# jimahlstrom/quisk

Hardware: AMD Instinct MI355X
Metric: Mcomplex-samples/s through RXA chain (higher is better)
Workload: dtype f64; 1 GPU; 256 channels/GPU x 192 kHz IQ -> 48 kHz SSB RXA chain (shift + 561-tap resample/4 + adc meter + NBP nc 2048 + S meter + fixed AGC + agc meter + panel), 2^22 input samples per channel per step; meters=on, ingest=f64, channels_per_gpu=256, total_channels=256, dsp_size=256, parallelism=channel-sharded x1 (weak), no collective

## Files before the change

### quisk_amd/csrc/qh_engine.hip

```cpp
#include <hip/hip_runtime.h>
#include <algorithm>
#include <cmath>
#include <cstdarg>
#include <cstdio>
#include <cstdlib>
#include <cstring>
#include <map>
#include <mutex>
#include <string>
#include <vector>
#include "../../include/quiskhip.h"
#include "qh_design.hpp"
#include "qh_kernels.hpp"
#include "qh_demod.hpp"
#include "qh_tiled.hpp"
#include "qh_agc_tiled.hpp"
#include "qh_emnr.hpp"
#include "qh_snba.hpp"
#include "qh_audio_peak.hpp"
#include "qh_ssql.hpp"
#include "qh_internal.hpp"

namespace qh {

thread_local std::string g_last_error;

int set_error(int code, const char *fmt, ...)
{
    char buf[512];
    va_list ap;
    va_start(ap, fmt);
    vsnprintf(buf, sizeof(buf), fmt, ap);
    va_end(ap);
    g_last_error = buf;
    return code;
}

static constexpr int kNfft = 4096;
static constexpr int kBandNfftMax = 8192;
static constexpr int kHistBand = 4095;
static constexpr int kLongPart = 4096, kLongNcMax = 65536, kLongParts = kLongNcMax / kLongPart, kLongHist = kLongNcMax - 1;
static constexpr int kHistFront = 2240;
static constexpr int kFmTile = 256;
static constexpr int kFmWarm = 768;
static constexpr int kSamTile = 4096;
static constexpr int kSamWarm = 8192;
static constexpr long long kSamTiledMin = 4 * 8192;
static constexpr int kAgcSegs = 16;
static constexpr long long kAgcTiledMin = 16384;

struct ChanCfg {
    int mode = QH_LSB;
    int shift_run = 1; double shift_freq = 0.0;
    int shift_on_device = 1;
    int nbp_run = 1, nbp_nc = 2048, nbp_wintype = 0;
    int mp = 0;
    std::vector<Notch> notches;
    double ndb_tunefreq = 0.0, ndb_shift = 0.0;
    int fnfrun = 0, autoincr = 1;
    double nbp_flow = -4150.0, nbp_fhigh = -150.0, nbp_gain = 1.0;
    int amd_run = 0, amd_mode = 0, fmd_run = 0;
// ... 395 lines not shown
    std::vector<cd> tw = fft_twiddle_table(kNfft);
    if (int rc = alloc(tw4096, (long long)tw.size())) return rc;
    if (int rc = upload(tw4096, tw, stream)) return rc;
    tw = fft_twiddle_table(kBandNfftMax);
    if (int rc = alloc(tw8192, (long long)tw.size())) return rc;
    if (int rc = upload(tw8192, tw, stream)) return rc;

    if (D > 1) {
        ResamplerDesign rd = design_resampler(in_rate, dsp_rate, 0.0, 0, 1.0);
        if (rd.L != 1 || rd.M != D) return set_error(QH_ERR_UNSUPPORTED, "resampler L/M = %d/%d not supported", rd.L, rd.M);
        front_ntaps = rd.ncoef;
        front_fold = D > 8 ? 8 : D;
        front_pick = D / front_fold;
        front_P = ((front_ntaps - 1 + front_fold - 1) / front_fold) * front_fold;
        front_L = (((kNfft - front_P) / front_fold) / front_pick) * front_pick;
        if (front_P > kHistFront) return set_error(QH_ERR_UNSUPPORTED, "resampler history %d too long", front_P);
        if (int rc = alloc(mask_front, (long long)nch * kNfft)) return rc;
        if (int rc = alloc(lane_rot, (long long)nch * NT)) return rc;
        if (int rc = alloc(front_taps, front_ntaps)) return rc;
        if (int rc = alloc(retune_list, nch)) return rc;
        if (int rc = alloc(retune_law, 2LL * nch)) return rc;
        QH_HIP(hipMemcpyAsync(front_taps, rd.h.data(), (size_t)front_ntaps * sizeof(double), hipMemcpyHostToDevice, stream));
        QH_HIP(hipStreamSynchronize(stream));
        QH_HIP(hipFuncSetAttribute(reinterpret_cast<const void *>(&front_mask_kernel<kNfft>), hipFuncAttributeMaxDynamicSharedMemorySize,
                                   (TileFft<kNfft, false, double2>::kLdsBytes)));
        std::vector<cd> twi = fft_twiddle_table(kNfft / front_fold);
        if (int rc = alloc(tw_inv_front, (long long)twi.size())) return rc;
        if (int rc = upload(tw_inv_front, twi, stream)) return rc;
        for (double2 *&h : hist_front) if (int rc = alloc(h, (long long)nch * kHistFront, true)) return rc;
    }
    if (int rc = alloc(mask_nbp, (long long)nch * kBandNfftMax)) return rc;
    if (int rc = alloc(mask_bp1, (long long)nch * kBandNfftMax)) return rc;
    for (int i = 0; i < 2; i++) {
        if (int rc = alloc(hist_nbp[i], (long long)nch * kHistBand, true)) return rc;
        if (int rc = alloc(hist_bp1[i], (long long)nch * kHistBand, true)) return rc;
    }
    if (int rc = alloc(nco_phase, nch, true)) return rc;
    if (int rc = alloc(nco_dphase, nch, true)) return rc;
    if (int rc = alloc(nco_parked, nch, true)) return rc;
    if (int rc = alloc(nco_step, nch)) return rc;
    if (int rc = alloc(epi, nch)) return rc;

#define QH_SET_LDS(D, ...) QH_HIP(hipFuncSetAttribute(reinterpret_cast<const void *>(&osfir_kernel<double, 4096, D, __VA_ARGS__>), \
                                                     hipFuncAttributeMaxDynamicSharedMemorySize, (osfir_lds_bytes<double, 4096, D, true>())))
    QH_SET_LDS(1, false); QH_SET_LDS(1, false, false, true);
    QH_SET_LDS(1, false, false, false, false, true); QH_SET_LDS(1, false, false, true, false, true);
#define QH_SET_LDS8(...) QH_HIP(hipFuncSetAttribute(reinterpret_cast<const void *>(&osfir_kernel<double, kBandNfftMax, 1, false, false, __VA_ARGS__>), \
                                                     hipFuncAttributeMaxDynamicSharedMemorySize, (osfir_lds_bytes<double, kBandNfftMax, 1, true>())))
    QH_SET_LDS8(false, false, false); QH_SET_LDS8(true, false, false); QH_SET_LDS8(false, false, true); QH_SET_LDS8(true, false, true);
#undef QH_SET_LDS8
#define QH_SET_LDS6K(...) QH_HIP(hipFuncSetAttribute(reinterpret_cast<const void *>(&osfir6k_kernel<__VA_ARGS__>), \
        hipFuncAttributeMaxDynamicSharedMemorySize, osfir6k_lds_bytes()))
    QH_SET_LDS6K(false, false); QH_SET_LDS6K(true, false); QH_SET_LDS6K(false, true); QH_SET_LDS6K(true, true);
#undef QH_SET_LDS6K
#define QH_SET_LDS2G(...) QH_HIP(hipFuncSetAttribute(reinterpret_cast<const void *>(&osfir8k_kernel<__VA_ARGS__>), \
                                                      hipFuncAttributeMaxDynamicSharedMemorySize, osfir8k_lds_bytes()))
    QH_SET_LDS2G(false, false); QH_SET_LDS2G(true, false); QH_SET_LDS2G(false, true); QH_SET_LDS2G(true, true);
#undef QH_SET_LDS2G
    QH_SET_LDS(2, false, false, false, true, false, true); QH_SET_LDS(4, false, false, false, true, false, true); QH_SET_LDS(8, false, false, false, true, false, true);
    QH_SET_LDS(2, false, true, false, true, false, true); QH_SET_LDS(4, false, true, false, true, false, true); QH_SET_LDS(8, false, true, false, true, false, true);
#undef QH_SET_LDS
    QH_HIP(hipStreamSynchronize(stream));
    return QH_OK;
}

static unsigned long long turns_fx(double f, double rate)
// ... 99 lines not shown
                } else {
                    h.assign(1, cd(1.0, 0.0));
                }
                last_bp1_h = h;
                if ((int)h.size() > kLongPart) h.resize((size_t)kLongPart);
                last_bp1 = band_mask(h);
                last_bp1_cfg = &c;
            }
            if (long_parts[1] > 1) if (int rc = long_masks_upload(1, ch, last_bp1_h)) return rc;
            if (int rc = put_mask(mask_bp1, ch, last_bp1)) return rc;
            c.bp1_dirty = false;
            lists_dirty = true;
        }
        if (c.nbp_flush) {
            if (int rc = zero_rows(hist_nbp, lhist[0], ch)) return rc;
            c.nbp_flush = false;
        }
        if (c.bp1_flush) {
            if (int rc = zero_rows(hist_bp1, lhist[1], ch)) return rc;
            c.bp1_flush = false;
        }
    }
    if (!nco_list.empty())
        hipLaunchKernelGGL((front_mask_kernel<kNfft>), dim3((unsigned)nco_list.size()), dim3(NT), (size_t)(TileFft<kNfft, false, double2>::kLdsBytes),
                           stream, (const double *)front_taps, front_ntaps, (const unsigned long long *)nco_dphase, (const int *)retune_list, front_fold,
                           (const double2 *)tw4096, mask_front, lane_rot, nco_step, 1);
    return QH_OK;
}

std::vector<cd> Engine::notched(const ChanCfg &c, double f_low, double f_high, double scale) const
{
    const double offset = c.ndb_tunefreq + c.ndb_shift;
    const double minwidth = (c.nbp_wintype == 1 ? 2200.0 : 1600.0) / (c.nbp_nc / 256) * ((double)dsp_rate / 48000);
    std::vector<std::pair<double, double>> bands = make_nbp(c.notches, minwidth, c.autoincr, f_low + offset, f_high + offset, nullptr);
    for (auto &b : bands) { b.first -= offset; b.second -= offset; }
    return fir_mbandpass(c.nbp_nc, bands, (double)dsp_rate, scale, c.nbp_wintype);
}

int Engine::snb_mask(ChanCfg &c, int ch)
{
    double f_low = 0.0, f_high = 0.0;
    int run_notches = 0;
    switch (c.mode) {
    case QH_LSB: case QH_CWL: case QH_DIGL: f_low = -5700.0; f_high = -250.0; run_notches = c.fnfrun; break;
    case QH_USB: case QH_CWU: case QH_DIGU: f_low = 250.0; f_high = 5700.0; run_notches = c.fnfrun; break;
    case QH_AM: case QH_SAM: case QH_DSB: case QH_FM: f_low = 250.0; f_high = 5700.0; break;
    default: break;
// ... 660 lines not shown
    QH_HIP(hipMemcpyAsync(emnr_GG, h_GG.data(), h_GG.size() * 8, hipMemcpyHostToDevice, stream));
    QH_HIP(hipMemcpyAsync(emnr_GGS, h_GGS.data(), h_GGS.size() * 8, hipMemcpyHostToDevice, stream));
    QH_HIP(hipMemcpyAsync(emnr_zeta, h_zeta.data(), h_zeta.size() * 8, hipMemcpyHostToDevice, stream));
    QH_HIP(hipMemcpyAsync(emnr_zeta_true, h_zeta_true.data(), h_zeta_true.size() * 4, hipMemcpyHostToDevice, stream));
    QH_HIP(hipStreamSynchronize(stream));
    QH_HIP(hipFuncSetAttribute(reinterpret_cast<const void *>(&emnr_kernel), hipFuncAttributeMaxDynamicSharedMemorySize, emnr_lds_bytes()));
    for (ChanCfg &c : cfg) { c.emnr_dirty = true; c.emnr_flush = false; }
    return QH_OK;
}

int Engine::ensure_buffers(long long n_mid)
{
    if (n_mid <= buf_cap) return QH_OK;
    if (int rc = quiesce()) return rc;
    for (double2 *&b : buf)
        if (int rc = alloc(b, n_mid * nch)) return rc;
    buf_cap = n_mid;
    return QH_OK;
}

std::vector<cd> Engine::band_mask(const std::vector<cd> &h) const
{
    std::vector<cd> m = make_mask(h, bnfft);
    if (!band2g) return m;
    std::vector<cd> p(m.size());
    const size_t half = m.size() / 2;
    for (size_t k = 0; k < half; k++) { p[k] = m[2 * k]; p[half + k] = m[2 * k + 1]; }
    return p;
}

int Engine::ensure_meter_partials(long long n_mid, int lout)
{
    const long long need = ((n_mid + lout - 1) / lout) * (lout / 64);
    if (need <= m_part_cap) return QH_OK;
    if (int rc = quiesce()) return rc;
    for (double2 *&m : m_part)
        if (int rc = alloc(m, need * nch)) return rc;
    m_part_cap = need;
    return QH_OK;
}

int Engine::ensure_abuf(long long n)
{
    return grow(abuf, abuf_cap, n, nch);
}

// ... 5 lines not shown
}

void Engine::tick(int cat)
{
    if (!timing) return;
    if (ev_used >= (int)ev.size()) {
        hipEvent_t e;
        (void)hipEventCreate(&e);
        ev.push_back(e);
        ev_cat.push_back(0);
    }
    ev_cat[(size_t)ev_used] = cat;
    (void)hipEventRecord(ev[(size_t)ev_used], stream);
    ev_used++;
}

template <int D, bool MIX, bool PACKED = false, bool METER = false, bool OUTMIX = false, bool EGRESS = false, int NFFT = kNfft, bool POLY = false,
          int DET = 0, bool PAIR = false>
static void launch_osfir(OsfirArgs<double> a, int ntiles, int nch, hipStream_t s)
{
    a.ntiles = ntiles;
    dim3 grid((unsigned)ntiles * (unsigned)nch), block(NT);
    constexpr int lds = osfir_lds_bytes<double, NFFT, D, METER>();
    hipLaunchKernelGGL((osfir_kernel<double, NFFT, D, MIX, PACKED, METER, OUTMIX, EGRESS, POLY, DET, PAIR>), grid, block, lds, s, a);
}
template <int NFFT>
static void launch_band(OsfirArgs<double> a, int ntiles, int nch, hipStream_t s, bool meter, bool egress)
{
    if (meter && egress) launch_osfir<1, false, false, true, false, true, NFFT>(a, ntiles, nch, s);
    else if (meter) launch_osfir<1, false, false, true, false, false, NFFT>(a, ntiles, nch, s);
    else if (egress) launch_osfir<1, false, false, false, false, true, NFFT>(a, ntiles, nch, s);
    else launch_osfir<1, false, false, false, false, false, NFFT>(a, ntiles, nch, s);
}

static void launch_band6k(OsfirArgs<double> a, int ntiles, int nch, hipStream_t s, bool meter, bool egress)
{
    a.ntiles = ntiles;
    dim3 grid((unsigned)ntiles * (unsigned)nch), block(kOsfir6kThreads);
    constexpr int lds = osfir6k_lds_bytes();
    if (meter && egress) hipLaunchKernelGGL((osfir6k_kernel<true, true>), grid, block, lds, s, a);
    else if (meter) hipLaunchKernelGGL((osfir6k_kernel<true, false>), grid, block, lds, s, a);
    else if (egress) hipLaunchKernelGGL((osfir6k_kernel<false, true>), grid, block, lds, s, a);
    else hipLaunchKernelGGL((osfir6k_kernel<false, false>), grid, block, lds, s, a);
}

static void launch_band2g(OsfirArgs<double> a, int ntiles, int nch, hipStream_t s, bool meter, bool egress)
{
// ... 2193 lines not shown
```

### quisk_amd/csrc/qh_fft.hpp

```cpp
#pragma once
#include <hip/hip_runtime.h>

namespace qh {

static constexpr double kThetaZeroMark = 8.0;


constexpr int NT = 256;

template <typename T> struct cplx_of;
template <> struct cplx_of<double> { using type = double2; };
template <> struct cplx_of<float>  { using type = float2; };
template <typename T> using cplx = typename cplx_of<T>::type;

template <typename T> __device__ __forceinline__ cplx<T> mk(T x, T y) { cplx<T> r; r.x = x; r.y = y; return r; }
template <typename C> __device__ __forceinline__ C cadd(C a, C b) { C r; r.x = a.x + b.x; r.y = a.y + b.y; return r; }
template <typename C> __device__ __forceinline__ C csub(C a, C b) { C r; r.x = a.x - b.x; r.y = a.y - b.y; return r; }
template <typename C> __device__ __forceinline__ C cmul(C a, C b)
{
    C r;
    r.x = a.x * b.x - a.y * b.y;
    r.y = a.x * b.y + a.y * b.x;
    return r;
}
__device__ __forceinline__ void lds_barrier()
{
    __builtin_amdgcn_fence(__ATOMIC_RELEASE, "workgroup", "local");
    __builtin_amdgcn_s_barrier();
    __builtin_amdgcn_fence(__ATOMIC_ACQUIRE, "workgroup", "local");
}

template <typename C> __device__ __forceinline__ C cconj(C a) { C r; r.x = a.x; r.y = -a.y; return r; }
template <bool INV, typename C> __device__ __forceinline__ C mul_mi(C a)
{
    C r;
    if (INV) { r.x = -a.y; r.y = a.x; } else { r.x = a.y; r.y = -a.x; }
    return r;
}

__device__ __forceinline__ constexpr double cos32(int a)
{
    constexpr double t[9] = { 1.0, 0.98078528040323044913, 0.92387953251128675613, 0.83146961230254523708,
                              0.70710678118654752440, 0.55557023301960222474, 0.38268343236508977173,
                              0.19509032201612826785, 0.0 };
    return t[a];
}

template <int R, int I, bool INV, typename C> __device__ __forceinline__ C mul_wconst(C a)
{
    using T = decltype(a.x);
    constexpr int A = I * (32 / R);
    if constexpr (A == 0) {
// ... 77 lines not shown
    for (int r = 2; r < R; r++) {
        if (r & 1) { wo = cmul(wo, w2); x[r] = cmul(x[r], wo); }
        else { x[r] = cmul(x[r], we); if (r + 2 < R) we = cmul(we, w2); }
    }
}

template <int N, int R, int Ns, bool INV, typename C, bool LEAN = false>
__device__ __forceinline__ int stockham_butterfly(C (&x)[R], int j, C w1)
{
    int k = j & (Ns - 1);
    if constexpr (Ns > 1) { if constexpr (LEAN) apply_twiddle_powers_lean<R>(x, w1); else apply_twiddle_powers<R>(x, w1); }
    Dft<R, INV, C>::run(x);
    return (j - k) * R + k;
}

template <int Ns, bool INV, typename C>
__device__ __forceinline__ C pass_twiddle(const C *__restrict__ tw_pass, int j)
{
    C w = tw_pass[j & (Ns - 1)];
    return INV ? cconj(w) : w;
}

template <int N, int R, bool INV, typename C>
__device__ __forceinline__ void pass_regs_to_lds(C (&x)[R], C *lds)
{
    static_assert(R == N / NT, "first pass radix must equal N/NT");
    const int j = threadIdx.x;
    Dft<R, INV, C>::run(x);
    if constexpr (16 % R == 0) {
        C *p = lds + lds_phys(j * R);
#pragma unroll
        for (int r = 0; r < R; r++) p[r] = x[r];
    } else {
        static_assert(R % 16 == 0, "first pass radix: a divisor or a multiple of 16");
        C *p = lds + lds_phys(j * R);
#pragma unroll
        for (int r = 0; r < R; r++) p[r + r / 16] = x[r];
    }
}

template <int N, int R> struct PassGeom {
    static constexpr int NB = N / R;
    static constexpr int PER = (NB + NT - 1) / NT;
};

template <int N, int R, int Ns, bool INV, typename C>
__device__ __forceinline__ void pass_lds_to_lds(C *lds, const C (&w1)[PassGeom<N, R>::PER])
{
    constexpr int NB = PassGeom<N, R>::NB;
    constexpr int PER = PassGeom<N, R>::PER;
    C x[PER][R];
    int base[PER];
    static_assert(NB % 16 == 0, "pass geometry");
#pragma unroll
    for (int p = 0; p < PER; p++) {
        int j = threadIdx.x + p * NT;
        if (NB >= NT || j < NB) {
            const C *q = lds + lds_phys(j);
#pragma unroll
            for (int r = 0; r < R; r++) x[p][r] = q[r * (NB + NB / 16)];
        }
    }
// ... 106 lines not shown
#pragma unroll
        for (int r = 0; r < 16; r++) x[r].y = rp[r * RS];
    }

    static __device__ __forceinline__ void run(C (&x)[16], void *lds_raw, const Tw &t) { run_at(x, lds_raw, t, threadIdx.x); }
    template <bool LEAN = false>
    static __device__ __forceinline__ void run_at(C (&x)[16], void *lds_raw, const Tw &t, int j)
    {
        T *lds = reinterpret_cast<T *>(lds_raw);
        Dft<16, INV, C>::run(x);
        if constexpr (kSwizzle) exchange_sw<1>(x, lds, j, 0);
        else exchange<1, 256 + 16 * kPad>(x, lds, (16 + kPad) * j, sphys(j));
        const int base = stockham_butterfly<4096, 16, 16, INV, C, LEAN>(x, j, t.a[0]);
        __syncthreads();
        if constexpr (kSwizzle) exchange_sw<2>(x, lds, j, base);
        else exchange<16 + kPad, 256 + 16 * kPad>(x, lds, sphys(base), sphys(j));
        stockham_butterfly<4096, 16, 256, INV, C, LEAN>(x, j, t.b);
    }

    template <int D>
    static __device__ __forceinline__ void run_poly(C (&x)[16], void *lds_raw, const Tw &t)
    {
        static_assert(!INV && (D == 2 || D == 4 || D == 8), "forward transform of a decimating stage");
        constexpr int R3 = 16 / D;
        const int j = threadIdx.x;
        T *lds = reinterpret_cast<T *>(lds_raw);
        Dft<16, INV, C>::run(x);
        if constexpr (kSwizzle) exchange_sw<1>(x, lds, j, 0);
        else exchange<1, 256 + 16 * kPad>(x, lds, (16 + kPad) * j, sphys(j));
        const int base = stockham_butterfly<4096, 16, 16, INV>(x, j, t.a[0]);
        __syncthreads();
        if constexpr (kSwizzle) exchange_sw<2>(x, lds, j, base);
        else exchange<16 + kPad, 256 + 16 * kPad>(x, lds, sphys(base), sphys(j));
        C w[R3];
        w[1] = t.b;
#pragma unroll
        for (int s = 1; s < D; s <<= 1) w[1] = cmul(w[1], w[1]);
#pragma unroll
        for (int r = 2; r < R3; r++) w[r] = (r & 1) ? cmul(w[r - 1], w[1]) : cmul(w[r / 2], w[r / 2]);
        C y[16];
#pragma unroll
        for (int a = 0; a < D; a++) {
            C b[R3];
            b[0] = x[a];
#pragma unroll
            for (int r = 1; r < R3; r++) b[r] = cmul(x[a + D * r], w[r]);
            Dft<R3, INV, C>::run(b);
#pragma unroll
            for (int r = 0; r < R3; r++) y[r + R3 * a] = b[r];
        }
#pragma unroll
        for (int r = 0; r < 16; r++) x[r] = y[r];
    }
};

constexpr int kFft6kThreads = 384;
constexpr int kFft6kPad = 2;
constexpr int kFft6kLdsBytes = (6144 + 6144 / 16 * kFft6kPad) * 8;

template <bool INV, typename C> __device__ __forceinline__ void dft3(C &a, C &b, C &c)
{
    const double h = 0.86602540378443864676;
    const C t1 = cadd(b, c);
    C t2; t2.x = a.x - 0.5 * t1.x; t2.y = a.y - 0.5 * t1.y;
    const C d = csub(b, c);
    C t3;
    if (INV) { t3.x = -h * d.y; t3.y = h * d.x; } else { t3.x = h * d.y; t3.y = -h * d.x; }
    a = cadd(a, t1);
    b = cadd(t2, t3);
    c = csub(t2, t3);
}

template <int M, bool INV, typename C> __device__ __forceinline__ C mul_w24(C a)
{
    constexpr int m = M % 24;
// ... 99 lines not shown
        }
        __syncthreads();
        if (mid) {
#pragma unroll
            for (int r = 0; r < 24; r++) w2[r * (16 + kPad)] = y[r].x;
        }
        __syncthreads();
        const double *r2 = lds + sphys(t);
#pragma unroll
        for (int r = 0; r < 16; r++) x[r].x = r2[r * (384 + 24 * kPad)];
        __syncthreads();
        if (mid) {
#pragma unroll
            for (int r = 0; r < 24; r++) w2[r * (16 + kPad)] = y[r].y;
        }
        __syncthreads();
#pragma unroll
        for (int r = 0; r < 16; r++) x[r].y = r2[r * (384 + 24 * kPad)];
        apply_twiddle_powers<16>(x, tw.last);
        Dft<16, INV, C>::run(x);
    }
};

template <int N, bool INV, typename C> struct TileFft {
    static constexpr bool kSplit = N == 4096 && sizeof(C) == 16;
    static constexpr int kLdsBytes = kSplit ? split4096_lds_bytes(8) : lds_elems<N>() * (int)sizeof(C);
    using Tw = typename FftRR<N, INV, C>::Tw;
    static __device__ __forceinline__ Tw load(const C *__restrict__ tw) { return FftRR<N, INV, C>::load(tw); }
    static __device__ __forceinline__ void run(C (&x)[N / NT], void *lds, const Tw &t)
    {
        if constexpr (kSplit) {
            FftSplit4096<INV, C>::run(x, lds, t);
        } else {
            FftRR<N, INV, C>::first(x, reinterpret_cast<C *>(lds));
            FftRR<N, INV, C>::rest(reinterpret_cast<C *>(lds), x, t);
        }
    }
    template <int D> static __device__ __forceinline__ void run_poly(C (&x)[N / NT], void *lds, const Tw &t)
    {
        static_assert(kSplit, "polyphase plan: the fp64 4096-point transform");
        FftSplit4096<INV, C>::template run_poly<D>(x, lds, t);
    }
};

template <bool INV, typename C> struct FftRR<2048, INV, C> {
    struct Tw { C a[2], b[1], c; };
    static __device__ __forceinline__ Tw load(const C *__restrict__ tw)
    {
        Tw t;
        t.a[0] = pass_twiddle<8, INV>(tw, threadIdx.x);
        t.a[1] = pass_twiddle<8, INV>(tw, threadIdx.x + NT);
        t.b[0] = pass_twiddle<32, INV>(tw + 8, threadIdx.x);
        t.c = pass_twiddle<256, INV>(tw + 40, threadIdx.x);
        return t;
    }
    static __device__ __forceinline__ void first(C (&x)[8], C *lds) { pass_regs_to_lds<2048, 8, INV>(x, lds); }
    static __device__ __forceinline__ void rest(C *lds, C (&x)[8], const Tw &t)
    {
        __syncthreads();
        pass_lds_to_lds<2048, 4, 8, INV>(lds, t.a);
        __syncthreads();
        pass_lds_to_lds<2048, 8, 32, INV>(lds, t.b);
        __syncthreads();
        pass_lds_to_regs<2048, 8, INV>(lds, x, t.c);
// ... 3 lines not shown
template <bool INV, typename C> struct FftRR<1024, INV, C> {
    struct Tw { C a[1], b[1], c[1], d; };
    static __device__ __forceinline__ Tw load(const C *__restrict__ tw)
    {
        Tw t;
        t.a[0] = pass_twiddle<4, INV>(tw, threadIdx.x);
        t.b[0] = pass_twiddle<16, INV>(tw + 4, threadIdx.x);
        t.c[0] = pass_twiddle<64, INV>(tw + 20, threadIdx.x);
        t.d = pass_twiddle<256, INV>(tw + 84, threadIdx.x);
        return t;
    }
    static __device__ __forceinline__ void first(C (&x)[4], C *lds) { pass_regs_to_lds<1024, 4, INV>(x, lds); }
    static __device__ __forceinline__ void rest(C *lds, C (&x)[4], const Tw &t)
    {
        __syncthreads();
        pass_lds_to_lds<1024, 4, 4, INV>(lds, t.a);
        __syncthreads();
        pass_lds_to_lds<1024, 4, 16, INV>(lds, t.b);
        __syncthreads();
        pass_lds_to_lds<1024, 4, 64, INV>(lds, t.c);
        __syncthreads();
        pass_lds_to_regs<1024, 4, INV>(lds, x, t.d);
    }
};

template <bool INV, typename C> struct FftRR<512, INV, C> {
    struct Tw { C a[1], b[1], c; };
    static __device__ __forceinline__ Tw load(const C *__restrict__ tw)
    {
        Tw t;
        t.a[0] = pass_twiddle<2, INV>(tw, threadIdx.x);
        t.b[0] = pass_twiddle<32, INV>(tw + 2, threadIdx.x);
        t.c = pass_twiddle<256, INV>(tw + 34, threadIdx.x);
        return t;
    }
    static __device__ __forceinline__ void first(C (&x)[2], C *lds) { pass_regs_to_lds<512, 2, INV>(x, lds); }
    static __device__ __forceinline__ void rest(C *lds, C (&x)[2], const Tw &t)
    {
        __syncthreads();
        pass_lds_to_lds<512, 16, 2, INV>(lds, t.a);
        __syncthreads();
        pass_lds_to_lds<512, 8, 32, INV>(lds, t.b);
        __syncthreads();
        pass_lds_to_regs<512, 2, INV>(lds, x, t.c);
    }
};
// ... 23 lines not shown
```

### quisk_amd/csrc/qh_kernels.hpp

```cpp
#pragma once
#include "qh_osfir.hpp"

namespace qh {

template <typename T, bool MIX, bool PACKED = false>
__global__ __launch_bounds__(NT) void hist_update_kernel(const cplx<T> *in, long long in_stride, int n_in,
                                                         const cplx<T> *old_hist, cplx<T> *new_hist, int H,
                                                         const unsigned long long *nco_phase,
                                                         const unsigned long long *nco_dphase,
                                                         const int *chan_list = nullptr,
                                                         const unsigned char *pk_src = nullptr, PackedFmt pk = PackedFmt{})
{
    using C = cplx<T>;
    const int ch = chan_list ? chan_list[blockIdx.y] : (int)blockIdx.y;
    const int j = blockIdx.x * NT + threadIdx.x;
    if (j >= H) return;
    const long long g = (long long)n_in - H + j;
    C v;
    if (g >= 0) {
        if constexpr (PACKED) v = decode_packed<T>(pk_src, pk, ch, g);
        else v = in[(long long)ch * in_stride + g];
        if constexpr (MIX) {
            unsigned long long ph = nco_phase[ch] + nco_dphase[ch] * (unsigned long long)g;
            C rot;
// ... 25 lines not shown
    if (tile >= ntiles) return;
    const long long g0 = g00 + (long long)tile * gstep;
    double2 r;
    sincos_turns<double>(phase[ch] + dphase[ch] * (unsigned long long)g0, r.x, r.y);
    tile_rot[(long long)ch * ntiles + tile] = r;
}

[[maybe_unused]] static __global__ void nco_retune_hist_kernel(double2 *hist, int H, const unsigned long long *phase,
                                                               const unsigned long long *dphase, const unsigned long long *parked,
                                                               const int *list, const unsigned long long *new_law)
{
    const int ch = list[blockIdx.y], j = blockIdx.x * blockDim.x + threadIdx.x;
    if (j >= H) return;
    const long long np = (long long)j - H;
    const unsigned long long act = new_law[2 * blockIdx.y], d_new = new_law[2 * blockIdx.y + 1];
    const unsigned long long p_new = act == 0 ? phase[ch] : act == 1 ? 0ull : parked[ch];
    const unsigned long long dphi = (phase[ch] - p_new) + (dphase[ch] - d_new) * (unsigned long long)np;
    double2 r;
    sincos_turns<double>(dphi, r.x, r.y);
    double2 *p = hist + (long long)ch * H + j;
    *p = cmul(*p, r);
}

template <int NFFT>
__global__ __launch_bounds__(NT) void front_mask_kernel(const double *taps, int ntaps, const unsigned long long *dphase, const int *list,
                                                        int D, const double2 *tw, double2 *mask, double2 *lane_rot, double2 *step, int poly)
{
    constexpr int E = NFFT / NT;
    using Fwd = TileFft<NFFT, false, double2>;
    extern __shared__ __align__(16) unsigned char smem_mask[];
    const int ch = list[blockIdx.x], t = threadIdx.x;
    const unsigned long long d = dphase[ch];
    double2 x[E];
#pragma unroll
    for (int r = 0; r < E; r++) {
        const int k = t + NT * r;
        x[r] = make_double2(0.0, 0.0);
        if (k < ntaps) {
            double c, s;
            sincos_turns<double>(0ull - d * (unsigned long long)k, c, s);
            const double h = taps[k];
            x[r] = make_double2(h * c, h * s);
        }
    }
    Fwd::run(x, smem_mask, Fwd::load(tw));
    if (poly) {
        const int EO = E / D;
        for (int i = 0; i < EO; i++)
            for (int a = 0; a < D; a++) {
                double2 acc = make_double2(0.0, 0.0);
                for (int q = 0; q < D; q++) {
                    double c, s;
                    sincospi(-2.0 * (double)((a * q) % D) / (double)D, &s, &c);
                    const double2 m = x[i + EO * q];
                    acc.x += m.x * c - m.y * s; acc.y += m.x * s + m.y * c;
                }
                double c, s;
                sincospi(-2.0 * (double)(((long long)a * (t + NT * i)) % NFFT) / (double)NFFT, &s, &c);
                mask[(long long)ch * NFFT + t + NT * (i + EO * a)] =
                    make_double2((acc.x * c - acc.y * s) * (1.0 / NFFT), (acc.x * s + acc.y * c) * (1.0 / NFFT));
            }
    } else {
#pragma unroll
        for (int r = 0; r < E; r++) mask[(long long)ch * NFFT + t + NT * r] = make_double2(x[r].x * (1.0 / NFFT), x[r].y * (1.0 / NFFT));
    }
    double2 lr;
    sincos_turns<double>(d * (unsigned long long)((long long)D * t), lr.x, lr.y);
    lane_rot[(long long)ch * NT + t] = lr;
    if (t == 0) {
        double2 st;
        sincos_turns<double>(d * (unsigned long long)((long long)D * NT), st.x, st.y);
        step[ch] = st;
    }
}

template <typename T, bool MIX, bool EGRESS = false>
__global__ __launch_bounds__(NT) void pointwise_kernel(const cplx<T> *in, long long in_stride, cplx<T> *out,
                                                       long long out_stride, int n,
                                                       const unsigned long long *nco_phase,
                                                       const unsigned long long *nco_dphase,
                                                       const EpiParam *epi, const int *chan_list = nullptr, EgressFmt eg = EgressFmt{})
{
    using C = cplx<T>;
    const int ch = chan_list ? chan_list[blockIdx.y] : (int)blockIdx.y;
    EpiParam ep;
    if (epi) ep = epi[ch]; else { ep.a = 1; ep.b = 0; ep.c = 0; ep.d = 1; }
    for (long long g = (long long)blockIdx.x * NT + threadIdx.x; g < n; g += (long long)gridDim.x * NT) {
// ... 17 lines not shown
```

### quisk_amd/csrc/qh_osfir.hpp

```cpp
#pragma once
#include "qh_fft.hpp"
#include "qh_wave.hpp"
#include "qh_ingest.hpp"
#include "qh_egress.hpp"

namespace qh {


struct EpiParam {
    double a, b, c, d;
};

template <typename T> struct OsfirArgs {
    const cplx<T> *in;
    const cplx<T> *hist;
    cplx<T> *hist_next;
    cplx<T> *out;
    const cplx<T> *mask;
    const cplx<T> *tw_fwd;
    const cplx<T> *tw_inv;
    const unsigned long long *nco_phase;
    const unsigned long long *nco_dphase;
    const double2 *nco_step;
    const EpiParam *epi;
// ... 113 lines not shown
{
    constexpr int a = TileFft<NFFT / U, false, cplx<T>>::kLdsBytes, b = TileFft<NFFT, true, cplx<T>>::kLdsBytes;
    return a > b ? a : b;
}

#ifndef QH_MASK_BATCH
#define QH_MASK_BATCH 8
#endif
#ifndef QH_OSFIR_WAVES_F64_D1
#define QH_OSFIR_WAVES_F64_D1 4
#endif
#ifndef QH_OSFIR_WAVES_F64
#define QH_OSFIR_WAVES_F64 3
#endif
#ifndef QH_OSFIR_WAVES_F64_OUTMIX
#define QH_OSFIR_WAVES_F64_OUTMIX 3
#endif
template <typename T, int D, bool OUTMIX = false, int NFFT = 4096> constexpr int osfir_min_waves()
{
    if (NFFT >= 8192) return sizeof(T) == 8 ? 1 : 2;
    return sizeof(T) == 8 ? (D == 1 ? QH_OSFIR_WAVES_F64_D1 : OUTMIX ? QH_OSFIR_WAVES_F64_OUTMIX : QH_OSFIR_WAVES_F64) : 4;
}

#ifdef QH_OSFIR_PROBE
__device__ long long g_osfir_probe[16];
#define QH_OPROBE(slot) do { if (blockIdx.x == 7 * 8 && threadIdx.x == 0) g_osfir_probe[slot] = clock64(); } while (0)
#else
#define QH_OPROBE(slot) do { } while (0)
#endif


template <int CTRL> __device__ __forceinline__ double dpp_mov_d(double v)
{
    int lo = __double2loint(v), hi = __double2hiint(v);
    lo = __builtin_amdgcn_mov_dpp(lo, CTRL, 0xf, 0xf, false);
    hi = __builtin_amdgcn_mov_dpp(hi, CTRL, 0xf, 0xf, false);
    return __hiloint2double(hi, lo);
}
constexpr int kMeterLdsDoublesPerWave = 2 * 64 * 9;

__device__ __forceinline__ double max_nn(double a, double b)
{
    double r;
    asm("v_max_f64 %0, %1, %2" : "=v"(r) : "v"(a), "v"(b));
    return r;
}
// ... 11 lines not shown
        for (int k = 0; k < 8; k++) {
            const C v = x[8 * g + k];
            double m2 = (double)v.x * (double)v.x;
            m2 = __builtin_fma((double)v.y, (double)v.y, m2);
            lds_wave[k * 72 + wr] = m2 * wlane;
            lds_wave[64 * 9 + k * 72 + wr] = m2;
        }
        __builtin_amdgcn_fence(__ATOMIC_RELEASE, "wavefront");
        __builtin_amdgcn_wave_barrier();
        __builtin_amdgcn_fence(__ATOMIC_ACQUIRE, "wavefront");
        double sum = rd[0], mx = rd[64 * 9];
#pragma unroll
        for (int k = 1; k < 8; k++) { sum += rd[k]; mx = max_nn(mx, rd[64 * 9 + k]); }
        sum += dpp_mov_d<0xB1>(sum); mx = max_nn(mx, dpp_mov_d<0xB1>(mx));
        sum += dpp_mov_d<0x4E>(sum); mx = max_nn(mx, dpp_mov_d<0x4E>(mx));
        sum += dpp_mov_d<0x141>(sum); mx = max_nn(mx, dpp_mov_d<0x141>(mx));
        const int r = 8 * g + (lane >> 3);
        if ((lane & 7) == 0 && r >= r0) dst[wave * ws + (r - r0)] = make_double2(sum, mx);
        __builtin_amdgcn_wave_barrier();
    }
}

template <typename T, int NFFT, int D, bool MIX, bool PACKED = false, bool METER = false, bool OUTMIX = false, bool EGRESS = false, bool POLY = false,
          int DET = 0, bool PAIR = false>
__global__ __launch_bounds__(NT, (osfir_min_waves<T, D, OUTMIX, NFFT>())) void osfir_kernel(OsfirArgs<T> a)
{
    using C = cplx<T>;
    constexpr int E = NFFT / NT;
    constexpr int NOUT = NFFT / D;
    constexpr int EO = E / D;
    static_assert(E % D == 0 && EO >= 1, "decimation must divide NFFT/256");
    static_assert(NOUT >= 2 * NT, "NFFT/D must be >= 512");
    static_assert(E <= 32, "validity bits are kept in one word");
    using Fwd = TileFft<NFFT, false, C>;
    using Inv = TileFft<NOUT, true, C>;
    extern __shared__ __align__(16) unsigned char smem[];
    void *lds = smem;

    const int t = threadIdx.x;
    int tile, slot;
    xcd_tile_map(a.ntiles, slot, tile);
    const int ch = PAIR ? a.chan_list[2 * slot] : a.chan_list ? a.chan_list[slot] : slot;
    const int ch_b = PAIR ? a.chan_list[2 * slot + 1] : ch;
    const C *in = a.in + (long long)ch * a.in_stride;
    const C *hist = a.hist ? a.hist + (long long)ch * a.hist_stride : nullptr;
    const int g0 = a.off - a.P + tile * (D * a.Lout);

    QH_OPROBE(0);
    C x[E];
    const bool interior = (g0 >= 0) && (g0 + NFFT <= a.n_in);
    if constexpr (PACKED) {
        const long long base = a.pk.first_offset + (long long)ch * a.pk.chan_stride + (long long)g0 * a.pk.record_stride;
        const bool fast = interior && a.pk.records_per_frame == 0 &&
                          base + (long long)(NFFT - 1) * a.pk.record_stride + 8 <= a.pk.total_bytes;
        if (fast) {
            const unsigned char *p = a.pk_src + base + (long long)t * a.pk.record_stride;
            const long long step = (long long)NT * a.pk.record_stride;
#pragma unroll
// ... 93 lines not shown
    }
    if constexpr (MIX) {
        C rot;
        sincos_turns<T>(a.nco_phase[ch] + a.nco_dphase[ch] * (unsigned long long)(long long)(g0 + t), rot.x, rot.y);
        const double2 st = a.nco_step[ch];
        const C step = mk<T>((T)st.x, (T)st.y);
        if (interior) {
#pragma unroll
            for (int r = 0; r < E; r++) { x[r] = cmul(x[r], rot); rot = cmul(rot, step); }
        } else {
#pragma unroll
            for (int r = 0; r < E; r++) {
                if (g0 + t + r * NT >= 0) x[r] = cmul(x[r], rot);
                rot = cmul(rot, step);
            }
        }
    }

    if constexpr (METER) {
        static_assert(D == 1 && !MIX && !PACKED, "meters ride on a plain D = 1 stage");
        static_assert(NT / 64 * kMeterLdsDoublesPerWave * 8 <= osfir_lds_bytes<T, NFFT, D, true>(), "meter blocks overlay the exchange image");
        meter_tap<C, E>(x, a.P >> 8, a.meter_w[t & 63], reinterpret_cast<double *>(lds) + (t >> 6) * kMeterLdsDoublesPerWave,
                        a.meter_in + (long long)ch * a.meter_stride + (long long)tile * (a.Lout >> 6), t >> 6, t & 63);
        __syncthreads();
    }

    QH_OPROBE(1);
    if constexpr (POLY) Fwd::template run_poly<D>(x, lds, Fwd::load(a.tw_fwd));
    else Fwd::run(x, lds, Fwd::load(a.tw_fwd));
    QH_OPROBE(2);

    const C *mask = a.mask + (long long)ch * a.mask_stride;
    C z[EO];
#pragma unroll
    for (int i = 0; i < EO; i++) {
        C acc = cmul(x[i], mask[t + NT * i]);
#pragma unroll
        for (int q = 1; q < D; q++) acc = cadd(acc, cmul(x[i + EO * q], mask[t + NT * (i + EO * q)]));
        z[i] = acc;
        if (((i + 1) * D) % QH_MASK_BATCH == 0) __builtin_amdgcn_sched_barrier(0);
    }

    QH_OPROBE(3);
    __syncthreads();
    Inv::run(z, lds, Inv::load(a.tw_inv));
    QH_OPROBE(4);
    if constexpr (METER) {
        __syncthreads();
        int t2 = t;
        asm volatile("" : "+v"(t2));
        meter_tap<C, EO>(z, a.P >> 8, a.meter_w[t2 & 63], reinterpret_cast<double *>(lds) + (t2 >> 6) * kMeterLdsDoublesPerWave,
                         a.meter_out + (long long)ch * a.meter_stride + (long long)tile * (a.Lout >> 6), t2 >> 6, t2 & 63);
    }

    if constexpr (OUTMIX) {
        static_assert(!MIX, "one oscillator");
        const double2 tr = a.tile_rot[(long long)ch * a.ntiles + tile];
        const double2 lr = a.lane_rot[(long long)ch * NT + t];
        const double2 st = a.nco_step[ch];
        C rot = cmul(mk<T>((T)tr.x, (T)tr.y), mk<T>((T)lr.x, (T)lr.y));
        const C step = mk<T>((T)st.x, (T)st.y);
#pragma unroll
        for (int i = 0; i < EO; i++) {
            z[i] = cmul(z[i], rot);
            if (i + 1 < EO) rot = cmul(rot, step);
        }
    }
// ... 428 lines not shown
```

Baseline: 146,100 Mcomplex-samples/s.

## Use swapped spectral order to keep FFT exchanges wavefront-private in fp64 4096 tile

Stores frequency-domain masks in a digit-swapped order within each 256-bin block, which the fp64 4096-point forward FFT now produces directly. One of its LDS exchanges then stays inside each wavefront, and the inverse starts from that same order. This lets several workgroup-wide __syncthreads be replaced by wavefront barriers, including the one after the meter tap and the one before the inverse transform. It adds new exchange code paths and a host-side permutation of band masks, and risks subtle correctness errors in the index mapping.

```diff
diff --git a/quisk_amd/csrc/qh_engine.hip b/quisk_amd/csrc/qh_engine.hip
--- a/quisk_amd/csrc/qh_engine.hip
+++ b/quisk_amd/csrc/qh_engine.hip
@@ -37,6 +37,12 @@
 }
 
 static constexpr int kNfft = 4096;
+static constexpr bool kSwap4096 = osfir_mask_layout<double, 4096, true>();
+template <int D, bool MIX = false, bool PACKED = false, bool METER = false, bool OUTMIX = false, bool EGRESS = false, bool POLY = false>
+static const void *engine_osfir4096()
+{
+    return reinterpret_cast<const void *>(&osfir_kernel<double, 4096, D, MIX, PACKED, METER, OUTMIX, EGRESS, POLY, 0, false, kSwap4096>);
+}
 static constexpr int kBandNfftMax = 8192;
 static constexpr int kHistBand = 4095;
 static constexpr int kLongPart = 4096, kLongNcMax = 65536, kLongParts = kLongNcMax / kLongPart, kLongHist = kLongNcMax - 1;
@@ -478,7 +484,7 @@
         if (int rc = alloc(retune_law, 2LL * nch)) return rc;
         QH_HIP(hipMemcpyAsync(front_taps, rd.h.data(), (size_t)front_ntaps * sizeof(double), hipMemcpyHostToDevice, stream));
         QH_HIP(hipStreamSynchronize(stream));
-        QH_HIP(hipFuncSetAttribute(reinterpret_cast<const void *>(&front_mask_kernel<kNfft>), hipFuncAttributeMaxDynamicSharedMemorySize,
+        QH_HIP(hipFuncSetAttribute(reinterpret_cast<const void *>(&front_mask_kernel<kNfft, kSwap4096>), hipFuncAttributeMaxDynamicSharedMemorySize,
                                    (TileFft<kNfft, false, double2>::kLdsBytes)));
         std::vector<cd> twi = fft_twiddle_table(kNfft / front_fold);
         if (int rc = alloc(tw_inv_front, (long long)twi.size())) return rc;
@@ -497,7 +503,7 @@
     if (int rc = alloc(nco_step, nch)) return rc;
     if (int rc = alloc(epi, nch)) return rc;
 
-#define QH_SET_LDS(D, ...) QH_HIP(hipFuncSetAttribute(reinterpret_cast<const void *>(&osfir_kernel<double, 4096, D, __VA_ARGS__>), \
+#define QH_SET_LDS(D, ...) QH_HIP(hipFuncSetAttribute(engine_osfir4096<D, __VA_ARGS__>(), \
                                                      hipFuncAttributeMaxDynamicSharedMemorySize, (osfir_lds_bytes<double, 4096, D, true>())))
     QH_SET_LDS(1, false); QH_SET_LDS(1, false, false, true);
     QH_SET_LDS(1, false, false, false, false, true); QH_SET_LDS(1, false, false, true, false, true);
@@ -643,7 +649,7 @@
         }
     }
     if (!nco_list.empty())
-        hipLaunchKernelGGL((front_mask_kernel<kNfft>), dim3((unsigned)nco_list.size()), dim3(NT), (size_t)(TileFft<kNfft, false, double2>::kLdsBytes),
+        hipLaunchKernelGGL((front_mask_kernel<kNfft, kSwap4096>), dim3((unsigned)nco_list.size()), dim3(NT), (size_t)(TileFft<kNfft, false, double2>::kLdsBytes),
                            stream, (const double *)front_taps, front_ntaps, (const unsigned long long *)nco_dphase, (const int *)retune_list, front_fold,
                            (const double2 *)tw4096, mask_front, lane_rot, nco_step, 1);
     return QH_OK;
@@ -1350,6 +1356,7 @@
 std::vector<cd> Engine::band_mask(const std::vector<cd> &h) const
 {
     std::vector<cd> m = make_mask(h, bnfft);
+    if (bnfft == kNfft) return spectral_layout<kSwap4096>(m);
     if (!band2g) return m;
     std::vector<cd> p(m.size());
     const size_t half = m.size() / 2;
@@ -1401,7 +1408,7 @@
     a.ntiles = ntiles;
     dim3 grid((unsigned)ntiles * (unsigned)nch), block(NT);
     constexpr int lds = osfir_lds_bytes<double, NFFT, D, METER>();
-    hipLaunchKernelGGL((osfir_kernel<double, NFFT, D, MIX, PACKED, METER, OUTMIX, EGRESS, POLY, DET, PAIR>), grid, block, lds, s, a);
+    hipLaunchKernelGGL((osfir_kernel<double, NFFT, D, MIX, PACKED, METER, OUTMIX, EGRESS, POLY, DET, PAIR, osfir_mask_layout<double, NFFT, true>()>), grid, block, lds, s, a);
 }
 template <int NFFT>
 static void launch_band(OsfirArgs<double> a, int ntiles, int nch, hipStream_t s, bool meter, bool egress)
diff --git a/quisk_amd/csrc/qh_fft.hpp b/quisk_amd/csrc/qh_fft.hpp
--- a/quisk_amd/csrc/qh_fft.hpp
+++ b/quisk_amd/csrc/qh_fft.hpp
@@ -1,5 +1,6 @@
 #pragma once
 #include <hip/hip_runtime.h>
+#include "qh_spectral.hpp"
 
 namespace qh {
 
@@ -28,6 +29,13 @@
     __builtin_amdgcn_fence(__ATOMIC_RELEASE, "workgroup", "local");
     __builtin_amdgcn_s_barrier();
     __builtin_amdgcn_fence(__ATOMIC_ACQUIRE, "workgroup", "local");
+}
+
+__device__ __forceinline__ void wave_lds_sync()
+{
+    __builtin_amdgcn_fence(__ATOMIC_RELEASE, "wavefront", "local");
+    __builtin_amdgcn_wave_barrier();
+    __builtin_amdgcn_fence(__ATOMIC_ACQUIRE, "wavefront", "local");
 }
 
 template <typename C> __device__ __forceinline__ C cconj(C a) { C r; r.x = a.x; r.y = -a.y; return r; }
@@ -151,10 +159,9 @@
 }
 
 template <int N, int R, bool INV, typename C>
-__device__ __forceinline__ void pass_regs_to_lds(C (&x)[R], C *lds)
+__device__ __forceinline__ void pass_regs_to_lds(C (&x)[R], C *lds, int j)
 {
     static_assert(R == N / NT, "first pass radix must equal N/NT");
-    const int j = threadIdx.x;
     Dft<R, INV, C>::run(x);
     if constexpr (16 % R == 0) {
         C *p = lds + lds_phys(j * R);
@@ -167,6 +174,8 @@
         for (int r = 0; r < R; r++) p[r + r / 16] = x[r];
     }
 }
+template <int N, int R, bool INV, typename C>
+__device__ __forceinline__ void pass_regs_to_lds(C (&x)[R], C *lds) { pass_regs_to_lds<N, R, INV>(x, lds, (int)threadIdx.x); }
 
 template <int N, int R> struct PassGeom {
     static constexpr int NB = N / R;
@@ -319,7 +328,6 @@
     static __device__ __forceinline__ void run_poly(C (&x)[16], void *lds_raw, const Tw &t)
     {
         static_assert(!INV && (D == 2 || D == 4 || D == 8), "forward transform of a decimating stage");
-        constexpr int R3 = 16 / D;
         const int j = threadIdx.x;
         T *lds = reinterpret_cast<T *>(lds_raw);
         Dft<16, INV, C>::run(x);
@@ -329,8 +337,14 @@
         __syncthreads();
         if constexpr (kSwizzle) exchange_sw<2>(x, lds, j, base);
         else exchange<16 + kPad, 256 + 16 * kPad>(x, lds, sphys(base), sphys(j));
+        poly_last<D>(x, t.b);
+    }
+    template <int D>
+    static __device__ __forceinline__ void poly_last(C (&x)[16], C tb)
+    {
+        constexpr int R3 = 16 / D;
         C w[R3];
-        w[1] = t.b;
+        w[1] = tb;
 #pragma unroll
         for (int s = 1; s < D; s <<= 1) w[1] = cmul(w[1], w[1]);
 #pragma unroll
@@ -348,6 +362,66 @@
         }
 #pragma unroll
         for (int r = 0; r < 16; r++) x[r] = y[r];
+    }
+
+    static constexpr int kWaveRegion = 64 * (16 + kPad);
+    static __device__ __forceinline__ void wave_sync() { wave_lds_sync(); }
+    static __device__ __forceinline__ void exchange_wave(C (&x)[16], T *lds, int l)
+    {
+        static_assert(!kSwizzle && kPad == 2, "the wavefronts' private quarters: the padded image, pitch 18");
+        constexpr int P = 16 + kPad;
+        T *wp = lds + P * ((l & ~0x18) | ((l & 8) << 1) | ((l & 16) >> 1));
+        const T *rp = lds + 32 * P * (l >> 5) + 8 * P * ((l >> 4) & 1) + (l & 15);
+#pragma unroll
+        for (int r = 0; r < 16; r++) wp[r] = x[r].x;
+        wave_sync();
+#pragma unroll
+        for (int r = 0; r < 16; r++) x[r].x = rp[16 * P * (r >> 3) + P * (r & 7)];
+        wave_sync();
+#pragma unroll
+        for (int r = 0; r < 16; r++) wp[r] = x[r].y;
+        wave_sync();
+#pragma unroll
+        for (int r = 0; r < 16; r++) x[r].y = rp[16 * P * (r >> 3) + P * (r & 7)];
+    }
+    static __device__ __forceinline__ Tw load_swapped(const C *__restrict__ tw)
+    {
+        return FftRR<4096, INV, C>::load_at(tw, INV ? (int)threadIdx.x : swap4((int)threadIdx.x));
+    }
+    template <int POLY_D = 1>
+    static __device__ __forceinline__ void run_fwd_swapped(C (&x)[16], void *lds_raw, const Tw &t)
+    {
+        static_assert(!INV, "forward transform");
+        T *lds = reinterpret_cast<T *>(lds_raw);
+        const int l = threadIdx.x;
+        Dft<16, INV, C>::run(x);
+        exchange<1, 256 + 16 * kPad>(x, lds, (16 + kPad) * l, sphys(swap4(l)));
+        apply_twiddle_powers<16>(x, t.a[0]);
+        Dft<16, INV, C>::run(x);
+        __syncthreads();
+        int l2 = l;
+        asm volatile("" : "+v"(l2));
+        exchange_wave(x, lds, l2);
+        if constexpr (POLY_D == 1) {
+            apply_twiddle_powers<16>(x, t.b);
+            Dft<16, INV, C>::run(x);
+        } else {
+            poly_last<POLY_D>(x, t.b);
+        }
+    }
+    static __device__ __forceinline__ void run_inv_swapped(C (&x)[16], void *lds_raw, const Tw &t)
+    {
+        static_assert(INV, "inverse transform");
+        T *lds = reinterpret_cast<T *>(lds_raw);
+        Dft<16, INV, C>::run(x);
+        int l = threadIdx.x;
+        asm volatile("" : "+v"(l));
+        exchange_wave(x, lds, l);
+        const int j = threadIdx.x;
+        const int base = stockham_butterfly<4096, 16, 16, INV>(x, j, t.a[0]);
+        __syncthreads();
+        exchange<16 + kPad, 256 + 16 * kPad>(x, lds, sphys(base), sphys(j));
+        stockham_butterfly<4096, 16, 256, INV>(x, j, t.b);
     }
 };
 
@@ -493,24 +567,38 @@
     }
 };
 
-template <int N, bool INV, typename C> struct TileFft {
+template <int N, bool INV, typename C, bool SWAP = false> struct TileFft {
     static constexpr bool kSplit = N == 4096 && sizeof(C) == 16;
-    static constexpr int kLdsBytes = kSplit ? split4096_lds_bytes(8) : lds_elems<N>() * (int)sizeof(C);
+    static_assert(!SWAP || INV || kSplit, "swapped forward transform: fp64, 4096 points");
+    static constexpr bool kPrivate1024 = SWAP && INV && N == 1024 && sizeof(C) == 16;
+    static constexpr bool kPrivateStart = (SWAP && INV && kSplit) || kPrivate1024;
+    static constexpr int kLdsBytes = kSplit ? split4096_lds_bytes(8) : kPrivate1024 ? 32000 : lds_elems<N>() * (int)sizeof(C);
     using Tw = typename FftRR<N, INV, C>::Tw;
-    static __device__ __forceinline__ Tw load(const C *__restrict__ tw) { return FftRR<N, INV, C>::load(tw); }
+    static __device__ __forceinline__ Tw load(const C *__restrict__ tw)
+    {
+        if constexpr (SWAP && kSplit) return FftSplit4096<INV, C>::load_swapped(tw);
+        else if constexpr (kPrivate1024) return FftRR<N, INV, C>::load_swapped(tw);
+        else return FftRR<N, INV, C>::load(tw);
+    }
     static __device__ __forceinline__ void run(C (&x)[N / NT], void *lds, const Tw &t)
     {
         if constexpr (kSplit) {
-            FftSplit4096<INV, C>::run(x, lds, t);
+            if constexpr (!SWAP) FftSplit4096<INV, C>::run(x, lds, t);
+            else if constexpr (INV) FftSplit4096<INV, C>::run_inv_swapped(x, lds, t);
+            else FftSplit4096<INV, C>::template run_fwd_swapped<1>(x, lds, t);
+        } else if constexpr (kPrivate1024) {
+            FftRR<N, INV, C>::run_swapped(x, reinterpret_cast<C *>(lds), t);
         } else {
-            FftRR<N, INV, C>::first(x, reinterpret_cast<C *>(lds));
+            if constexpr (SWAP) pass_regs_to_lds<N, N / NT, INV>(x, reinterpret_cast<C *>(lds), swap4((int)threadIdx.x));
+            else FftRR<N, INV, C>::first(x, reinterpret_cast<C *>(lds));
             FftRR<N, INV, C>::rest(reinterpret_cast<C *>(lds), x, t);
         }
     }
     template <int D> static __device__ __forceinline__ void run_poly(C (&x)[N / NT], void *lds, const Tw &t)
     {
         static_assert(kSplit, "polyphase plan: the fp64 4096-point transform");
-        FftSplit4096<INV, C>::template run_poly<D>(x, lds, t);
+        if constexpr (SWAP) FftSplit4096<INV, C>::template run_fwd_swapped<D>(x, lds, t);
+        else FftSplit4096<INV, C>::template run_poly<D>(x, lds, t);
     }
 };
 
@@ -560,6 +648,42 @@
         __syncthreads();
         pass_lds_to_regs<1024, 4, INV>(lds, x, t.d);
     }
+    static constexpr int kWaveStride = 64 * (16 + QH_SPLIT_PAD) / 2;
+    static constexpr int kSwappedLdsBytes = (3 * kWaveStride + 4 * 68) * 16 > lds_elems<1024>() * 16 ? (3 * kWaveStride + 4 * 68) * 16 : lds_elems<1024>() * 16;
+    static __device__ __forceinline__ Tw load_swapped(const C *__restrict__ tw)
+    {
+        Tw t = load(tw);
+        t.a[0] = pass_twiddle<4, INV>(tw, ((int)threadIdx.x >> 2) & 3);
+        return t;
+    }
+    static __device__ __forceinline__ void run_swapped(C (&x)[4], C *lds, const Tw &t)
+    {
+        static_assert(INV && sizeof(C) == 16, "the fp64 inverse behind FftSplit4096::run_fwd_swapped");
+        static_assert(kSwappedLdsBytes <= split4096_lds_bytes(8), "the regions lie inside the 4096-point transform's image");
+        Dft<4, INV, C>::run(x);
+        int l = threadIdx.x;
+        asm volatile("" : "+v"(l));
+        C *region = lds + kWaveStride * (l >> 6);
+        C *wp = region + (l & 63);
+        const C *rp = region + 68 * ((l >> 2) & 3) + (l & 51);
+#pragma unroll
+        for (int q = 0; q < 4; q++) wp[68 * q] = x[q];
+        wave_lds_sync();
+#pragma unroll
+        for (int r = 0; r < 4; r++) x[r] = rp[4 * r];
+        const int j = ((l >> 2) & 3) + 4 * (l >> 4) + 64 * (l & 3);
+        const int base = stockham_butterfly<1024, 4, 4, INV>(x, j, t.a[0]);
+        __syncthreads();
+        C *q = lds + lds_phys(base);
+#pragma unroll
+        for (int r = 0; r < 4; r++) q[4 * r] = x[r];
+        __syncthreads();
+        pass_lds_to_lds<1024, 4, 16, INV>(lds, t.b);
+        __syncthreads();
+        pass_lds_to_lds<1024, 4, 64, INV>(lds, t.c);
+        __syncthreads();
+        pass_lds_to_regs<1024, 4, INV>(lds, x, t.d);
+    }
 };
 
 template <bool INV, typename C> struct FftRR<512, INV, C> {
diff --git a/quisk_amd/csrc/qh_kernels.hpp b/quisk_amd/csrc/qh_kernels.hpp
--- a/quisk_amd/csrc/qh_kernels.hpp
+++ b/quisk_amd/csrc/qh_kernels.hpp
@@ -71,7 +71,7 @@
     *p = cmul(*p, r);
 }
 
-template <int NFFT>
+template <int NFFT, bool SWAP = false>
 __global__ __launch_bounds__(NT) void front_mask_kernel(const double *taps, int ntaps, const unsigned long long *dphase, const int *list,
                                                         int D, const double2 *tw, double2 *mask, double2 *lane_rot, double2 *step, int poly)
 {
@@ -106,12 +106,12 @@
                 }
                 double c, s;
                 sincospi(-2.0 * (double)(((long long)a * (t + NT * i)) % NFFT) / (double)NFFT, &s, &c);
-                mask[(long long)ch * NFFT + t + NT * (i + EO * a)] =
+                mask[(long long)ch * NFFT + spectral_slot<SWAP>(t + NT * (i + EO * a))] =
                     make_double2((acc.x * c - acc.y * s) * (1.0 / NFFT), (acc.x * s + acc.y * c) * (1.0 / NFFT));
             }
     } else {
 #pragma unroll
-        for (int r = 0; r < E; r++) mask[(long long)ch * NFFT + t + NT * r] = make_double2(x[r].x * (1.0 / NFFT), x[r].y * (1.0 / NFFT));
+        for (int r = 0; r < E; r++) mask[(long long)ch * NFFT + spectral_slot<SWAP>(t + NT * r)] = make_double2(x[r].x * (1.0 / NFFT), x[r].y * (1.0 / NFFT));
     }
     double2 lr;
     sincos_turns<double>(d * (unsigned long long)((long long)D * t), lr.x, lr.y);
diff --git a/quisk_amd/csrc/qh_osfir.hpp b/quisk_amd/csrc/qh_osfir.hpp
--- a/quisk_amd/csrc/qh_osfir.hpp
+++ b/quisk_amd/csrc/qh_osfir.hpp
@@ -159,6 +159,8 @@
     return sizeof(T) == 8 ? (D == 1 ? QH_OSFIR_WAVES_F64_D1 : OUTMIX ? QH_OSFIR_WAVES_F64_OUTMIX : QH_OSFIR_WAVES_F64) : 4;
 }
 
+template <typename T, int NFFT, bool ENGINE> constexpr bool osfir_mask_layout() { return QH_SPECTRAL_SWAP != 0 && ENGINE && sizeof(T) == 8 && NFFT == 4096; }
+
 #ifdef QH_OSFIR_PROBE
 __device__ long long g_osfir_probe[16];
 #define QH_OPROBE(slot) do { if (blockIdx.x == 7 * 8 && threadIdx.x == 0) g_osfir_probe[slot] = clock64(); } while (0)
@@ -216,7 +218,7 @@
 }
 
 template <typename T, int NFFT, int D, bool MIX, bool PACKED = false, bool METER = false, bool OUTMIX = false, bool EGRESS = false, bool POLY = false,
-          int DET = 0, bool PAIR = false>
+          int DET = 0, bool PAIR = false, bool SWAP = false>
 __global__ __launch_bounds__(NT, (osfir_min_waves<T, D, OUTMIX, NFFT>())) void osfir_kernel(OsfirArgs<T> a)
 {
     using C = cplx<T>;
@@ -226,8 +228,9 @@
     static_assert(E % D == 0 && EO >= 1, "decimation must divide NFFT/256");
     static_assert(NOUT >= 2 * NT, "NFFT/D must be >= 512");
     static_assert(E <= 32, "validity bits are kept in one word");
-    using Fwd = TileFft<NFFT, false, C>;
-    using Inv = TileFft<NOUT, true, C>;
+    static_assert(!SWAP || (sizeof(T) == 8 && NFFT == 4096), "swapped spectral side: the fp64 4096-point tile");
+    using Fwd = TileFft<NFFT, false, C, SWAP>;
+    using Inv = TileFft<NOUT, true, C, SWAP>;
     extern __shared__ __align__(16) unsigned char smem[];
     void *lds = smem;
 
@@ -367,7 +370,8 @@
         static_assert(NT / 64 * kMeterLdsDoublesPerWave * 8 <= osfir_lds_bytes<T, NFFT, D, true>(), "meter blocks overlay the exchange image");
         meter_tap<C, E>(x, a.P >> 8, a.meter_w[t & 63], reinterpret_cast<double *>(lds) + (t >> 6) * kMeterLdsDoublesPerWave,
                         a.meter_in + (long long)ch * a.meter_stride + (long long)tile * (a.Lout >> 6), t >> 6, t & 63);
-        __syncthreads();
+        static_assert(kMeterLdsDoublesPerWave == 64 * (16 + QH_SPLIT_PAD) || !SWAP, "a wavefront's meter block is its quarter of the image");
+        if constexpr (!SWAP) __syncthreads();
     }
 
     QH_OPROBE(1);
@@ -387,7 +391,7 @@
     }
 
     QH_OPROBE(3);
-    __syncthreads();
+    if constexpr (!Inv::kPrivateStart) __syncthreads();
     Inv::run(z, lds, Inv::load(a.tw_inv));
     QH_OPROBE(4);
     if constexpr (METER) {
diff --git a/quisk_amd/csrc/qh_spectral.hpp b/quisk_amd/csrc/qh_spectral.hpp
--- /dev/null
+++ b/quisk_amd/csrc/qh_spectral.hpp
@@ -0,0 +1,28 @@
+#pragma once
+#include <cstddef>
+
+#if defined(__HIPCC__) || defined(__CUDACC__)
+#define QH_SPECTRAL_HD __host__ __device__
+#else
+#define QH_SPECTRAL_HD
+#endif
+
+#ifndef QH_SPECTRAL_SWAP
+#define QH_SPECTRAL_SWAP 1
+#endif
+
+namespace qh {
+
+QH_SPECTRAL_HD constexpr int swap4(int l) { return ((l & 15) << 4) | ((l >> 4) & 15); }
+
+template <bool SWAP> QH_SPECTRAL_HD constexpr int spectral_slot(int k) { return SWAP ? (k & ~255) | swap4(k & 255) : k; }
+
+template <bool SWAP, typename V> V spectral_layout(const V &natural)
+{
+    if (!SWAP) return natural;
+    V p(natural.size());
+    for (size_t k = 0; k < natural.size(); k++) p[(size_t)spectral_slot<SWAP>((int)k)] = natural[k];
+    return p;
+}
+
+}
```

Result: slower. 144,000 Mcomplex-samples/s (-1.4%).
